# snap-research/F8Net

Hardware: AMD Instinct MI355X
Metric: images/sec at bs=128 (ResNet-50 INT8) (higher is better)
Workload: dtype int8 x int8 -> int32 (exact integer)

## Files before the change

f8net_amd/_lib.py:

```python
import ctypes
import os

_HERE = os.path.dirname(os.path.abspath(__file__))
LIB_PATH = os.environ.get('F8NET_LIB') or os.path.join(_HERE, 'libf8net.so')

F8_OK = 0


class F8Error(RuntimeError):
    def __init__(self, status, msg):
        super().__init__(f'libf8net: {msg} (status {status})')
        self.status = status


class ConvDesc(ctypes.Structure):
    _fields_ = [(n, ctypes.c_int32) for n in
                ('cin', 'cout', 'kernel', 'stride', 'pad', 'groups', 'weight_fl', 'input_fl',
                 'input_signed', 'quant_input', 'relu')]


class LinearDesc(ctypes.Structure):
    _fields_ = [(n, ctypes.c_int32) for n in
                ('in_features', 'out_features', 'weight_fl', 'input_fl', 'input_signed', 'quant_input')]

# ... 25 lines not shown
    ('f8_net_num_launches', _i, [_vp]),
    ('f8_net_arena_bytes', _sz, [_vp]),
    ('f8_net_weight_bytes', _sz, [_vp]),
    ('f8_net_output_fraclen', _i, [_vp]),
    ('f8_net_output_elems', _sz, [_vp]),
    ('f8_net_upload', _i, [_vp]),
    ('f8_net_num_parts', _i, [_vp, _i]),
    ('f8_net_step_launches', _i, [_vp, _i, _i]),
    ('f8_net_run', _i, [_vp, _vp, _vp, _i, _vp]),
    ('f8_net_run_f32', _i, [_vp, _vp, _i, _vp, _i, _vp]),
    ('f8_net_run_u8', _i, [_vp, _vp, _i, _i, ctypes.POINTER(ctypes.c_float), ctypes.POINTER(ctypes.c_float), _vp, _i, _vp]),
    ('f8_net_run_profiled', _i, [_vp, _vp, _vp, _i, _vp, ctypes.POINTER(ctypes.c_float), _i]),
    ('f8_net_launch_info', _i, [_vp, _i, _i, ctypes.c_char_p, _sz, ctypes.POINTER(ctypes.c_double),
                                ctypes.POINTER(ctypes.c_double)]),
    ('f8_net_launch_kernel', _i, [_vp, _i, ctypes.c_char_p, _sz]),
    ('f8_net_launch_valu', _i, [_vp, _i, _i, ctypes.POINTER(ctypes.c_double)]),
    ('f8_net_set_label', _i, [_vp, _i, ctypes.c_char_p]),
    ('f8_net_set_pipelined', _i, [_vp, _i]),
    ('f8_net_autotune', _i, [_vp, _i, _vp]),
    ('f8_net_set_option', _i, [_vp, ctypes.c_char_p, _i]),
    ('f8_net_get_option', _i, [_vp, ctypes.c_char_p, ctypes.POINTER(_i)]),
    ('f8_net_set_input_ready', _i, [_vp, _vp]),
    ('f8_net_check', _i, [_vp]),
]


def lib():
    global _lib
    if _lib is None:
        if not os.path.exists(LIB_PATH):
# ... 18 lines not shown
```

f8net_amd/csrc/f8_chain.hip:

```cpp
#include "f8_device.h"
#include <cstdio>
#include <cstdlib>

namespace f8 {

template <int C, int MID, int W, int H, int R, int CIN0, bool BROT_ = false, bool ALIAS_ = false>
struct ChainCfg {
    static constexpr bool BROT = BROT_, ALIAS = ALIAS_;
    static constexpr int BSLOTS = BROT ? 2 : kChainMaxBlocks;
    static constexpr int T = (H + R - 1) / R;
    static constexpr int PX = R * W, NPT = (PX + 31) / 32, ROWS = NPT * 32;
    static constexpr int PW = W + 2, PR = R + 2;
    static constexpr int XS = C + 16, MS = MID + 16, IS = CIN0 + 16;
    static constexpr int X8_BYTES = ROWS * XS;
    static constexpr int PATCH_BYTES = (PR * PW * MS + 255) / 256 * 256;
    static constexpr int MID2_BYTES = ROWS * MS;
    static constexpr int XIN_BYTES = CIN0 != C ? ROWS * IS : 0;
    static constexpr int BIAS_INTS = 2 * MID + C;
    static constexpr int BIAS_BYTES = (BSLOTS * BIAS_INTS + (CIN0 != C ? C : 0)) * 4;
    static constexpr int MISC_BYTES = 256;
    static_assert(!ALIAS || XIN_BYTES <= PATCH_BYTES, "ALIAS: the shortcut's operand fits the patch");
    static constexpr int LDS_BYTES = X8_BYTES + PATCH_BYTES + MID2_BYTES + (ALIAS ? 0 : XIN_BYTES) + BIAS_BYTES + MISC_BYTES;
    static constexpr int ROWB = W * MID;
    static_assert(LDS_BYTES <= 160 * 1024, "LDS");
    static_assert(X8_BYTES < 65536 + 4096 && PATCH_BYTES < 65536 && MID2_BYTES < 65536, "immediate offsets");
    static_assert(ROWB / 16 <= 256 && (size_t)512 * 4 * ROWB <= kChainXchgBytes, "one 16-byte piece of a halo row per thread of a half workgroup");
};

template <int FAST, bool ACC = false>
__device__ __forceinline__ v4i quant_tile16(const v16i& y, int n, int lo, int hi, unsigned x_or) {
    unsigned d[4];
    const float sc = FAST == 1 ? requant_u8_scale(n) : 0.0f;
#pragma unroll
    for (int g = 0; g < 4; ++g) {
        if constexpr (FAST == 1) d[g] = requant_u8x4(y[4 * g], y[4 * g + 1], y[4 * g + 2], y[4 * g + 3], sc) ^ x_or;
        else if constexpr (FAST == 2) d[g] = requant_u8x4_int(y[4 * g], y[4 * g + 1], y[4 * g + 2], y[4 * g + 3], n) ^ x_or;
        else d[g] = pack4(requant1(y[4 * g], n, lo, hi), requant1(y[4 * g + 1], n, lo, hi), requant1(y[4 * g + 2], n, lo, hi), requant1(y[4 * g + 3], n, lo, hi)) ^ x_or;
    }
    auto s0 = __builtin_amdgcn_permlane32_swap(d[0], d[2], false, false);
// ... 27 lines not shown
#ifndef F8_CH_PRIO
#define F8_CH_PRIO 0
#endif
#ifndef F8_CH_BREG
#define F8_CH_BREG 1
#endif
    constexpr bool EARLY = F8_CH_EARLY != 0 && T > 1 && !ROT;
#ifndef F8_CH_SPLIT
#define F8_CH_SPLIT 1
#endif
#ifndef F8_CH_HALO_AUX
#define F8_CH_HALO_AUX 17
#endif
    constexpr int PG_ = NW / (MID / 32), NPW_ = ((R * W + 31) / 32 + PG_ - 1) / PG_;
    constexpr bool SPLIT = F8_CH_SPLIT != 0 && EARLY && PG_ >= 2 && T * R == H && W <= NPW_ * 32 && (R - 1) * W >= NPW_ * 32;
    static_assert(NB <= CM && CM % NB == 0 && NK1 % NB == 0, "a batch of K steps stays inside one 3x3 tap / one weight tile");
    static_assert(!DS0 || KS % NB == 0, "stage-opening block: whole batches");
    static_assert(!ROT || (NK1 % 8 == 0 && CM == 8), "rotation: groups of 8 K steps (256 bytes of a row), whole taps");
    static_assert(WSTAT || NPT == 2, "streamed P3: exactly one pixel pair");
    static_assert(W <= 62, "tile");

    if constexpr (FAST == 1) set_fp_round_nearest_even();
    extern __shared__ __attribute__((aligned(16))) char lds[];
    char* const x8 = lds;
    char* const patch = x8 + Cfg::X8_BYTES;
    char* const mid2 = patch + Cfg::PATCH_BYTES;
    char* const xin = Cfg::ALIAS ? patch : mid2 + Cfg::MID2_BYTES;
    int* const bias_lds = (int*)(mid2 + Cfg::MID2_BYTES + (Cfg::ALIAS ? 0 : Cfg::XIN_BYTES));
    int* const misc = bias_lds + Cfg::BIAS_BYTES / 4;

// ... 31 lines not shown
    auto bias_store = [&](int b, const int (&v)[NBI]) {
        int tb = tid; asm volatile("" : "+v"(tb));
#pragma unroll
        for (int k = 0; k < NBI; ++k) if (tb + k * NT < BIAS_INTS) bias_lds[(b & 1) * BIAS_INTS + tb + k * NT] = v[k];
    };
    if constexpr (!BROT) {
        for (int b = 0; b < a.nblk; ++b) {
            const ChainBlk& B = a.blk[b];
            for (int i = tid; i < BIAS_INTS; i += NT)
                bias_lds[b * BIAS_INTS + i] = i < 2 * MID ? ((TAIL && b == 0) ? 0 : (i < MID ? B.b0[i] : B.b2[i - MID])) : B.b4[i - 2 * MID];
        }
    }
    if constexpr (DS0) for (int i = tid; i < C; i += NT) bias_lds[BSLOTS * BIAS_INTS + i] = a.blk[0].bsc[i];
    __syncthreads();
    const int L = __builtin_amdgcn_readfirstlane(misc[0]);
    const int grp = L / T, ti = L - grp * T;
    const int p0 = ti * R;
    const int rows = (H - p0) < R ? (H - p0) : R;
    const int npx = rows * W;
    const bool has_up = ti > 0, has_dn = ti < T - 1;
    const int rot = ROT ? __builtin_amdgcn_readfirstlane(L * 5 + wave * 3) : 0;

    unsigned* const flags = a.sync + 16;
    const unsigned long long t_limit = (unsigned long long)a.timeout_ticks;
#ifdef F8_TRACE
    unsigned long long tt[16] = {}; unsigned long long t_prev = __builtin_readcyclecounter();
#define F8_CT(i) do { const unsigned long long now_ = __builtin_readcyclecounter(); tt[i] += now_ - t_prev; t_prev = now_; } while (0)
#else
#define F8_CT(i)
#endif

    const int mt = wave & (CM - 1), pg = wave / CM;
    v16i res[NPT][CTW];
    v4i wbuf[NBUF][NB];
    unsigned seq = 0;
// ... 38 lines not shown
            const int f = BI * NB + s, I = f / (NPAIR * KT2), k = f % KT2;
            dst[s] = k < KS ? ldw(wsc, (I * KS + k) * 1024, (unsigned)(wave * CTW * KS * 1024) + wl) : ldw(w4, (I * KK + (k - KS)) * 1024, (unsigned)(wave * CTW * KK * 1024) + wl);
        }
    };
    auto pin = [](auto& xf) {
#pragma unroll
        for (int j = 0; j < (int)(sizeof(xf) / sizeof(xf[0])); ++j) asm volatile("" : "+v"(xf[j]));
    };

    constexpr int CHX = CIN0 / 16, CHM = MID / 16;
    constexpr int NXI = DS0 ? (NPT * 32 * CHX + NT - 1) / NT : 0, NMI = TAIL ? (NPT * 32 * CHM + NT - 1) / NT : 0;
    v4i vin[NXI + NMI > 0 ? NXI + NMI : 1];
    auto in_issue = [&](int n, bool live) {
        if constexpr (DS0) {
            int tq0 = tid; asm volatile("" : "+v"(tq0));
            const int mt0 = (n * H + p0) * W;
#pragma unroll
            for (int k = 0; k < NXI; ++k) {
                const int idx = tq0 + k * NT, row = idx / CHX, c16 = idx % CHX;
                vin[k] = v4i{0, 0, 0, 0};
                if constexpr (TAIL) {
                    const int pr = row / W, pc = row - pr * W;
                    if (live && row < npx) vin[k] = *(const v4i*)(a.x8in + ((size_t)(n * 2 * H + 2 * (p0 + pr)) * (2 * W) + 2 * pc) * CIN0 + c16 * 16);
                } else {
                    if (live && row < npx) vin[k] = *(const v4i*)(a.x8in + (size_t)(mt0 + row) * CIN0 + c16 * 16);
                }
            }
#pragma unroll
            for (int k = 0; k < NMI; ++k) {
                const int idx = tq0 + k * NT, row = idx / CHM, c16 = idx % CHM;
                vin[NXI + k] = v4i{0, 0, 0, 0};
                if (live && row < npx) vin[NXI + k] = *(const v4i*)(a.m2in + (size_t)(mt0 + row) * MID + c16 * 16);
            }
        }
    };
    auto in_commit = [&]() {
        if constexpr (DS0) {
            int tq0 = tid; asm volatile("" : "+v"(tq0));
#pragma unroll
            for (int k = 0; k < NXI; ++k) { const int idx = tq0 + k * NT; if (idx < NPT * 32 * CHX) *(v4i*)(xin + (idx / CHX) * IS + (idx % CHX) * 16) = vin[k]; }
#pragma unroll
            for (int k = 0; k < NMI; ++k) { const int idx = tq0 + k * NT; if (idx < NPT * 32 * CHM) *(v4i*)(mid2 + (idx / CHM) * MS + (idx % CHM) * 16) = vin[NXI + k]; }
        }
    };
#ifndef F8_CH_PREFETCH
#define F8_CH_PREFETCH 1
#endif
    if (F8_CH_PREFETCH) in_issue(grp < a.N ? grp : 0, grp < a.N);

    for (int n = grp; n < a.N; n += a.NG) {
        const int m_tile = (n * H + p0) * W;
        if (!F8_CH_PREFETCH) in_issue(n, true);

        if constexpr (TAIL) {
            static_assert(KT2 % NB == 0 && KS % NB == 0 && NPT % 2 == 0, "TAIL: whole batches per K loop, pixel-tile pairs");
            int bv0[NBI], bv1[NBI];
            if constexpr (BROT) { bias_fetch(0, bv0); bias_fetch(a.nblk > 1 ? 1 : 0, bv1); }
            { F8_LANES; static_for<(NBUF - 1 < NBT ? NBUF - 1 : NBT)>([&](auto bc) { constexpr int Bi = decltype(bc)::value; wt_load(a.blk[0].wsc, a.blk[0].w4, wbuf[Bi], bc, wl16); }); }
            if constexpr (BROT) { bias_store(0, bv0); bias_store(1, bv1); }
            in_commit();
        } else if constexpr (!DS0) {
            F8_LANES;
            const ChainBlk& B0 = a.blk[0];
            const __amdgpu_buffer_rsrc_t rxr = __builtin_amdgcn_make_buffer_rsrc((void*)a.xr, 0, (unsigned)(((a.N * H * W + 31) & ~31) * C * 4), 0x00020000);
#pragma unroll
            for (int pt = 0; pt < NPT; ++pt) {
// ... 79 lines not shown
#define F8_CH_BFILL 1
#endif
                    {
                        const v4i zv = {(int)xor1, (int)xor1, (int)xor1, (int)xor1};
                        if constexpr (F8_CH_BFILL) {
                            constexpr int RB = PW * MS, CPM = MS / 16;
                            for (int o = tq_ * 16; o < RB; o += NT * 16) *(v4i*)(patch + o) = zv;
                            for (int o = (rows + 1) * RB + tq_ * 16; o < Cfg::PR * RB; o += NT * 16) *(v4i*)(patch + o) = zv;
                            if (tq_ < rows * 2 * CPM) {
                                const int r = tq_ / (2 * CPM), q = tq_ - r * 2 * CPM, sidec = q / CPM, c16 = q - sidec * CPM;
                                *(v4i*)(patch + ((r + 1) * PW + (sidec ? PW - 1 : 0)) * MS + c16 * 16) = zv;
                            }
                        } else {
                            for (int o = tq_ * 16; o < Cfg::PATCH_BYTES; o += NT * 16) *(v4i*)(patch + o) = zv;
                        }
                    }
                    v16i acc[NPW];
#pragma unroll
                    for (int g = 0; g < 4; ++g) {
                        const v4i bv = *(const v4i*)(bl + mt * 32 + 8 * g + 4 * lh);
#pragma unroll
                        for (int j = 0; j < NPW; ++j)
#pragma unroll
                            for (int e = 0; e < 4; ++e) acc[j][4 * g + e] = bv[e];
                    }
                    F8_CT(6);
                    constexpr int NBAT1 = NK1B / NB;
                    const char* const xsrc = DSB ? xin : x8;
                    auto rd = [&](v4i (&xf)[NPW], auto gc) {
                        constexpr int G = decltype(gc)::value;
// ... 130 lines not shown
                            for (int e = 0; e < 4; ++e) acc[j][4 * g + e] = bv[e];
                    }
                    unsigned bpb[NPW];
#pragma unroll
                    for (int j = 0; j < NPW; ++j) {
                        const int pix = p12_pix[j], oc = pix < npx ? pix : npx - 1;
                        const int orow = oc / W, ocol = oc - orow * W;
                        bpb[j] = (unsigned)((orow * PW + ocol) * MS + lh * 16);
                    }
                    v4i xfa[NPW], xfb[NPW];
                    constexpr int GH = SPLIT ? 6 * CM : (EARLY ? 3 * CM : NK2 + 1);
                    const int ord = (SPLIT && !((pg + 1) * NPW * 32 > (R - 1) * W)) ? 1 : 0;
                    unsigned bpb2[NPW], bpb3[NPW];
#pragma unroll
                    for (int j = 0; j < NPW; ++j) { bpb2[j] = bpb[j] + (unsigned)(ord ? 2 * PW * MS : 0); bpb3[j] = bpb[j] + (unsigned)(ord ? 0 : 2 * PW * MS); }
                    auto rd = [&](v4i (&xf)[NPW], auto gc) {
                        constexpr int G = decltype(gc)::value, TAP0 = G / CM, CI = G % CM;
                        if constexpr (SPLIT) {
                            constexpr int GRP = TAP0 / 3, DX = TAP0 % 3;
#pragma unroll
                            for (int j = 0; j < NPW; ++j) {
                                if constexpr (GRP == 0) xf[j] = *(const v4i*)(patch + bpb[j] + (PW + DX) * MS + CI * 32);
                                else if constexpr (GRP == 1) xf[j] = *(const v4i*)(patch + bpb2[j] + DX * MS + CI * 32);
                                else xf[j] = *(const v4i*)(patch + bpb3[j] + DX * MS + CI * 32);
                            }
                        } else {
                            constexpr int TAP = EARLY ? (TAP0 < 3 ? TAP0 + 3 : (TAP0 < 6 ? TAP0 - 3 : TAP0)) : TAP0;
                            if constexpr (ROT) {
                                const int tp = tap_of(TAP);
                                const int tr = tp / 3, ts = tp - tr * 3;
                                const unsigned eo = (unsigned)((tr * PW + ts) * MS + CI * 32);
#pragma unroll
                                for (int j = 0; j < NPW; ++j) xf[j] = *(const v4i*)(patch + bpb[j] + eo);
                            } else {
#pragma unroll
                                for (int j = 0; j < NPW; ++j) xf[j] = *(const v4i*)(patch + bpb[j] + ((TAP / 3) * PW + TAP % 3) * MS + CI * 32);
                            }
                        }
                    };
                    rd(xfa, std::integral_constant<int, 0>{});
                    static_for<NK2>([&](auto gc) {
                        constexpr int G = decltype(gc)::value, Bi = G / NB, S = G % NB;
                        if constexpr (S == 0 && Bi + NBUF - 1 < NBAT2) w2_load(pw2, wbuf[(Bi + NBUF - 1) % NBUF], Bi + NBUF - 1, wl16, ord);
                        v4i (&cur)[NPW] = (G & 1) ? xfb : xfa;
                        v4i (&nxt)[NPW] = (G & 1) ? xfa : xfb;
                        if constexpr (G == GH) { F8_CT(3); consume(); F8_CT(2); rd(cur, gc); }
                        if constexpr (G + 1 < NK2 && G + 1 != GH) rd(nxt, std::integral_constant<int, G + 1>{});
                        pin(cur);
#pragma unroll
                        for (int j = 0; j < NPW; ++j) acc[j] = __builtin_amdgcn_mfma_i32_32x32x32_i8(wbuf[Bi % NBUF][S], cur[j], acc[j], 0, 0, 0);
                    });
// ... 182 lines not shown
            }
        };
#ifndef F8_CH_PEEL_LAST
#define F8_CH_PEEL_LAST 1
#endif
        if constexpr (TAIL) block(0, std::integral_constant<int, 2>{}, std::integral_constant<int, 2>{});
        else if constexpr (DS0) block(0, std::integral_constant<int, 1>{}, std::integral_constant<int, 2>{});
        if constexpr (F8_CH_PEEL_LAST) {
            const int b0 = DS0 ? 1 : 0;
            for (int b = b0; b + 1 < a.nblk; ++b) block(b, std::integral_constant<int, 0>{}, std::integral_constant<int, 0>{});
            if (a.nblk > b0) block(a.nblk - 1, std::integral_constant<int, 0>{}, std::integral_constant<int, 1>{});
        } else {
            for (int b = DS0 ? 1 : 0; b < a.nblk; ++b) block(b, std::integral_constant<int, 0>{}, std::integral_constant<int, 2>{});
        }

        if (F8_CH_PREFETCH) in_issue(n + a.NG < a.N ? n + a.NG : n, n + a.NG < a.N);
        if (a.q[0].ptr) {
            constexpr int CH = C / 16;
            int tq1 = tid; asm volatile("" : "+v"(tq1));
            for (int idx = tq1; idx < npx * CH; idx += NT) {
                const int row = idx / CH, c16 = idx % CH;
                const v4i v = *(const v4i*)(x8 + row * XS + c16 * 16);
                *(v4i*)(a.q[0].ptr + (size_t)(m_tile + row) * C + c16 * 16) = v;
            }
        }
        __syncthreads();
        F8_CT(5);
    }
    if (tid == 0) {
        asm volatile("s_waitcnt vmcnt(0)" ::: "memory");
        misc[2] = (__hip_atomic_fetch_add(a.sync + 1, 1u, __ATOMIC_RELAXED, __HIP_MEMORY_SCOPE_AGENT) == gridDim.x - 1u) ? 1 : 0;
// ... 33 lines not shown
void chain_shape(int C, int MID, int H, int W, int cin0, bool tail, int* R, int* wg_per_cu) {
    *R = 4; *wg_per_cu = 1;
    if (F8_CH_R2_S0 && !tail && C == 256 && MID == 64 && H == 56 && W == 56 && cin0 == 64) { *R = 2; *wg_per_cu = 2; }
    if (chain_nw(C, MID, H, W, cin0, tail) == 4) { *R = 2; *wg_per_cu = 2; }
}

template <int C, int MID, int W, int H, int R, int CIN0, int NB, int NBUF, int FAST, bool ROT, bool TAIL = false, int NW = 8>
static hipError_t launch_chain_t(const ChainArgs& a, hipStream_t s) {
    using Cfg = ChainCfg<C, MID, W, H, R, CIN0, TAIL || R < 4, TAIL && NW == 4>;
    static unsigned long long attr_done = 0; int attr_dev = -1;
    if (!dyn_lds_opted_in(&attr_done, &attr_dev)) {
        hipError_t e = hipFuncSetAttribute((const void*)chain_kernel<C, MID, W, H, R, CIN0, NB, NBUF, FAST, ROT, TAIL, NW>, hipFuncAttributeMaxDynamicSharedMemorySize, Cfg::LDS_BYTES);
        if (e != hipSuccess) return e;
        if (attr_dev >= 0) attr_done |= 1ull << attr_dev;
    }
    const int grid = a.NG * Cfg::T;
    if (grid < 1 || grid > (R < 4 ? 512 : 256)) return hipErrorInvalidValue;
#ifdef F8_TRACE
    static unsigned long long* tbuf = nullptr; static int count = 0;
    static const int want = [] { const char* e = getenv("F8_TRACE_CHAIN"); return e ? atoi(e) : -1; }();
    ChainArgs b = a;
    const bool tracing = (count++ == want);
    if (tracing) { if (!tbuf) (void)hipMalloc((void**)&tbuf, (size_t)1 << 19); (void)hipMemsetAsync(tbuf, 0, (size_t)grid * 1024, s); b.trace = tbuf; }
    hipLaunchKernelGGL((chain_kernel<C, MID, W, H, R, CIN0, NB, NBUF, FAST, ROT, TAIL, NW>), dim3(grid), dim3(NW * 64), Cfg::LDS_BYTES, s, b);
    if (tracing) {
        (void)hipStreamSynchronize(s);
        static unsigned long long hb[256 * 8 * 16];
        (void)hipMemcpy(hb, tbuf, (size_t)grid * 1024, hipMemcpyDeviceToHost);
        double ph[16] = {}, pw[8][16] = {}; int n = 0;
        for (int i = 0; i < grid; ++i) {
            ++n;
// ... 36 lines not shown
        if (!(a.q[0].n > 0 && a.q[0].n <= 30 && a.q[0].lo == 0)) return 0;
        f16 = f16 && a.q[0].n <= kRequantU8MaxShift;
    }
    return (a.rq_int || !a.acc_ok || !a.stream_ok || !f16) ? 2 : 1;
}

#define F8_STR2(...) #__VA_ARGS__
#define F8_STR(...) F8_STR2(__VA_ARGS__)
static bool chain_rot(int H, bool tail) {
#ifdef F8_CH_ROT
    return H == 14 && !tail;
#else
    (void)H; (void)tail; return false;
#endif
}
int chain_kernel_name(char* buf, size_t cap, int C, int MID, int H, int W, int cin0, bool tail, int fast) {
    if (cchain_supported(C, MID, H, W, cin0, tail)) return cchain_kernel_name(buf, cap, fast);
    int R = 4, wg = 1;
    chain_shape(C, MID, H, W, cin0, tail, &R, &wg);
    const char* nb = MID == 64 ? F8_STR(F8_CH_S0) : (MID == 128 ? F8_STR(F8_CH_S1) : F8_STR(F8_CH_S2));
    return snprintf(buf, cap, "f8::chain_kernel<%d, %d, %d, %d, %d, %d, %s, %d, %s, %s, %d>", C, MID, W, H, R, cin0, nb, fast, chain_rot(H, tail) ? "true" : "false", tail ? "true" : "false",
                    chain_nw(C, MID, H, W, cin0, tail));
}

hipError_t launch_chain(const ChainArgs& a, int fast, int C, int MID, int H, int W, int cin0, hipStream_t s) {
    if (a.nblk < 1 || a.nblk > kChainMaxBlocks) return hipErrorInvalidValue;
    if (cchain_supported(C, MID, H, W, cin0, a.tail != 0)) return launch_cchain(a, fast, s);
#define F8_CHAIN_INST(...) (fast == 1 ? launch_chain_t<__VA_ARGS__, 1, F8_CHAIN_ROT>(a, s) : fast == 2 ? launch_chain_t<__VA_ARGS__, 2, F8_CHAIN_ROT>(a, s) : launch_chain_t<__VA_ARGS__, 0, F8_CHAIN_ROT>(a, s))
#define F8_CHAIN_ROT false
#if F8_CH_R2_S0
// ... 37 lines not shown
```

f8net_amd/csrc/f8_internal.h:

```cpp
#pragma once
#include <hip/hip_runtime.h>
#include <stdint.h>
#include <stddef.h>

namespace f8 {

struct Options {
    int split = 2;
    int fuse_blocks = 1;
    int fuse_stages = -1;
    int fuse_dual = 1;
    int fuse_ds = 1;
    int fuse_opener = 1;
    int fuse_fc = 1;
    int fuse_stem = 1;
    int fuse_input = 1;
    int wstat = 1;
    int wstat_min_tiles = 2;
    int wstat_fast = 1;
    int s2wreg = 1;
    int wreg = 1;
    int fuse_bchain = 2;
    int fuse_chain = 1;
    int fuse_chain7 = 1;
    int fuse_pool = 1;
    int fuse_tail = 1;
    int chain_timeout_ms = 10000;
    int fuse_p12 = 1;
    int fuse_head2 = 1;
    int fuse_ir = 1;
    int fuse_irchain = 0;
    int patch3x3 = 1;
    int dual_wide = 2048;
    int deep_nk = 7;
    int bk128 = 0;
    int dw_dot4 = 1;
    int dw_mma = 1;
    int stem_rows = 1;
    int stem_grid_div = 0;
    int stem_wpc = 3;
    int opener_stg = 1;
    int chunk56 = -1, chunk28 = -1, chunk14 = -1;
// ... 137 lines not shown

    const int32_t* xr;
    const int8_t* x8in;
    const int8_t* m2in; int32_t tail;
    int32_t N, NG;
    int32_t* out32; QuantOut q[2];
    uint32_t* sync;
    uint32_t* err;
    uint32_t* err_host;
    uint32_t epoch;
    int8_t* xchg;
    uint32_t timeout_ticks;
    void* trace;
    int32_t R;
    int32_t pool;
};
constexpr int kChainSyncWords = 16 + 512;
constexpr int kChainErrWord = 1000;
constexpr size_t kChainXchgBytes = (size_t)512 * 2 * 2 * 3584;

struct BChainBlk {
    const int8_t* wa; const int8_t* wb;
    const int32_t* ba; const int32_t* bb;
    int32_t nq, loq, hiq; uint32_t xorq;
    int32_t n1, lo1, hi1; uint32_t xor1;
    int32_t relu_a, relu1;
    int32_t acc_shl, res_shl;
};
constexpr int kBChainMaxBlocks = 6;
struct BChainArgs {
// ... 94 lines not shown
int conv_inst(const ConvArgs& a, const ConvTile& t, bool res, bool dual, int deep_nk);
int conv_kernel_name(char* buf, size_t cap, const ConvArgs& a, const ConvTile& t, int inst);
hipError_t launch_conv(const ConvArgs& a, const ConvTile& t, int inst, hipStream_t s);
hipError_t launch_fused_bottleneck(const FusedArgs& a, hipStream_t s);
int fused_bottleneck_kernel_name(char* buf, size_t cap, const FusedArgs& a);
bool fused_bottleneck_supported(int C, int MID, int H, int W, int imgs_per_launch, int stage_mask, int* R);
bool fused_ds_supported(int C, int MID, int COUT, int H, int W, int* R);
bool fused_opener_supported(int C, int MID, int COUT, int H, int W, int* R);
int fused_opener_inst(const FusedArgs& a, bool stg);
int fused_opener_kernel_name(char* buf, size_t cap, const FusedArgs& a, int inst);
hipError_t launch_fused_opener(const FusedArgs& a, int inst, hipStream_t s);
bool chain_supported(int C, int MID, int H, int W, int cin0);
bool chain_tail_supported(int C, int MID, int H, int W, int cin0);
int chain_max_blocks(int C, int MID, int H, int W, int cin0, bool tail);
void chain_shape(int C, int MID, int H, int W, int cin0, bool tail, int* R, int* wg_per_cu);
hipError_t launch_chain(const ChainArgs& a, int fast, int C, int MID, int H, int W, int cin0, hipStream_t s);
int chain_kernel_name(char* buf, size_t cap, int C, int MID, int H, int W, int cin0, bool tail, int fast);
bool cchain_supported(int C, int MID, int H, int W, int cin0, bool tail);
size_t cchain_xchg_bytes();
int cchain_clusters(int N, int slots);
int cchain_kernel_name(char* buf, size_t cap, int fast);
int chain_fast(const ChainArgs& a, unsigned shortcut_blocks, bool q8);
hipError_t launch_cchain(const ChainArgs& a, int fast, hipStream_t s);
bool bchain_supported(int C, int H, int W);
bool bchain_ds_supported(int C, int H, int W);
int bchain_tiles_per_img(int C, int H, int W);
hipError_t launch_bchain(const BChainArgs& a, int fast, int C, int H, int W, hipStream_t s);
int bchain_fast(const BChainArgs& a, bool ds, bool q8);
int bchain_kernel_name(char* buf, size_t cap, int C, int H, int W, bool ds, int fast);
bool fused_p12_supported(int C, int MID, int H, int W);
// ... 61 lines not shown
```

f8net_amd/csrc/f8_net.cpp:

```cpp
#include "../../include/f8net.h"
#include "f8_internal.h"

#include <algorithm>
#include <cstdarg>
#include <cstdio>
#include <cstdlib>
#include <cstring>
#include <new>
#include <variant>
#include <string>
#include <mutex>
#include <vector>

using namespace f8;

namespace {

thread_local std::string g_err;

int fail(int code, const char* fmt, ...) {
    char buf[512];
    va_list ap;
    va_start(ap, fmt);
    vsnprintf(buf, sizeof buf, fmt, ap);
// ... 236 lines not shown
    {"fuse_ds", "F8_FUSE_DS", &Options::fuse_ds, 0, 1, true},
    {"fuse_opener", "F8_FUSE_OPENER", &Options::fuse_opener, 0, 1, true},
    {"fuse_fc", "F8_FUSE_FC", &Options::fuse_fc, 0, 1, true},
    {"fuse_stem", "F8_FUSE_STEM", &Options::fuse_stem, 0, 1, true},
    {"fuse_input", "F8_FUSE_INPUT", &Options::fuse_input, 0, 1, true},
    {"fuse_ir", "F8_FUSE_IR", &Options::fuse_ir, 0, 2, true},
    {"fuse_irchain", "F8_FUSE_IRCHAIN", &Options::fuse_irchain, 0, 1, true},
    {"fuse_head2", "F8_FUSE_HEAD2", &Options::fuse_head2, 0, 1, true},
    {"fuse_p12", "F8_FUSE_P12", &Options::fuse_p12, 0, 1, true},
    {"fuse_chain", "F8_FUSE_CHAIN", &Options::fuse_chain, 0, 1, true},
    {"fuse_tail", "F8_FUSE_TAIL", &Options::fuse_tail, 0, 1, true},
    {"fuse_chain7", "F8_FUSE_CHAIN7", &Options::fuse_chain7, 0, 1, true},
    {"fuse_pool", "F8_FUSE_POOL", &Options::fuse_pool, 0, 1, true},
    {"fuse_bchain", "F8_FUSE_BCHAIN", &Options::fuse_bchain, 0, 2, true},
    {"chain_timeout_ms", "F8_CHAIN_TIMEOUT_MS", &Options::chain_timeout_ms, 0, 1 << 20, false},
    {"wreg", "F8_WREG", &Options::wreg, 0, 1, true},
    {"s2wreg", "F8_S2WREG", &Options::s2wreg, 0, 1, true},
    {"wstat", "F8_WSTAT", &Options::wstat, 0, 1, true},
    {"wstat_min_tiles", "F8_WSTAT_MIN_TILES", &Options::wstat_min_tiles, 0, 1 << 20, true},
    {"wstat_fast", "F8_WSTAT_FAST", &Options::wstat_fast, 0, 1, true},
    {"patch3x3", "F8_PATCH3X3", &Options::patch3x3, 0, 1, true},
    {"dual_wide", "F8_DUAL_WIDE", &Options::dual_wide, 0, 1 << 30, true},
    {"deep_nk", "F8_DEEP_NK", &Options::deep_nk, 1, 1 << 20, true},
    {"bk128", "F8_BK128", &Options::bk128, 0, 1, true},
    {"dw_dot4", "F8_DW_DOT4", &Options::dw_dot4, 0, 1, true},
    {"dw_mma", "F8_DW_MMA", &Options::dw_mma, 0, 1, true},
    {"stem_wpc", "F8_STEM_WPC", &Options::stem_wpc, 1, 8, false},
    {"stem_rows", "F8_STEM_ROWS", &Options::stem_rows, 0, 1, true},
    {"stem_grid_div", "F8_STEM_GRID_DIV", &Options::stem_grid_div, 0, 32, false},
    {"opener_stg", "F8_OPENER_STG", &Options::opener_stg, 0, 1, true},
// ... 1880 lines not shown
                B.relu_a = na.cd.relu; B.relu_b = nb.cd.relu; B.relu1 = ND[hh.fused_add].relu;
                if (k == 0) { a.acc_ok = 1; a.rq_int = rq_int; a.stream_ok = (hds || stream_bounded(net, na.a)) ? 1 : 0; }
                a.acc_ok = a.acc_ok && conv_acc_bounded(na) && conv_acc_bounded(nb);
                a.stream_ok = a.stream_ok && stream_bounded(net, ND[hh.fused_add].out);
                const int dfl = T[hh.out].fl - (hds ? T[ng.out].fl : T[na.a].fl);
                B.acc_shl = dfl < 0 ? -dfl : 0; B.res_shl = dfl > 0 ? dfl : 0;
            }
            const Node& hf = ND[ch[0]];
            const bool tail = hf.tail, ds = hf.fbd_a >= 0 || tail;
            const Node& a0 = tail ? ND[hf.dual] : ND[ds ? hf.fbd_a : hf.fb_a];
            const Tensor& oT = T[ND[nd.fused_add].out];
            a.tail = tail ? 1 : 0;
            a.pool = nd.pool >= 0 ? 1 : 0;
            st.C = oT.C; st.MID = tail ? a0.cd.cin : a0.cd.cout; st.H = oT.H; st.W = oT.W; st.cin0 = tail ? hf.cd.cin : a0.cd.cin;
            chain_shape(st.C, st.MID, st.H, st.W, st.cin0, tail, &a.R, &st.wg_per_cu);
            st.tiles = (st.H + a.R - 1) / a.R;
            st.cluster = (!ds || tail) && cchain_supported(st.C, st.MID, st.H, st.W, st.cin0, tail);
            out_formats(a.q);
            st.inst = chain_fast(a, shortcut_blocks, nq > 0);
            chain_kernel_name(kb, sizeof kb, st.C, st.MID, st.H, st.W, st.cin0, tail, st.inst);
            st.args = a; break;
        }
        case S_BCHAIN: {
            const std::vector<int>& ch = nd.bchain;
            BChainArgs a{};
            a.nblk = (int)ch.size();
            const bool ds = ND[ch[0]].bds_a >= 0;
            for (int k = 0; k < a.nblk; ++k) {
                const Node& hk = ND[ch[k]];
                const bool hds = hk.bds_a >= 0;
                const Node& c2 = hds ? ND[hk.bds_b] : hk; Node& c1 = ND[hds ? hk.bds_a : hk.bb_a];
                BChainBlk& B = a.blk[k];
// ... 233 lines not shown
            if ((e = hipMalloc((void**)&net->d_chain, net->chain_stride * parts_cap)) != hipSuccess) return hip_fail(e, "hipMalloc(chain scratch)");
            if ((e = hipMemset(net->d_chain, 0, net->chain_stride * parts_cap)) != hipSuccess) return hip_fail(e, "hipMemset(chain scratch)");
            if (hipHostMalloc((void**)&net->h_err, 64, hipHostMallocMapped) == hipSuccess) {
                *net->h_err = 0u;
                if (hipHostGetDevicePointer((void**)&net->h_err_dev, net->h_err, 0) != hipSuccess) { (void)hipHostFree(net->h_err); net->h_err = nullptr; net->h_err_dev = nullptr; }
            } else { net->h_err = nullptr; (void)hipGetLastError(); }
        }
    for (int p = 0; p < parts_cap; ++p)
        if (net->stem_zero_bytes && (e = hipMemset(net->d_arena + p * net->arena_stride + net->stem_zero_off, net->stem_zero_val, net->stem_zero_bytes)) != hipSuccess)
            return hip_fail(e, "hipMemset(stem halo)");
    if ((e = hipDeviceSynchronize()) != hipSuccess) return hip_fail(e, "upload sync");
    net->uploaded = true;
    return F8_OK;
}

static int chain_launch_groups(const f8_net* net, const Step& st, int N) {
    const int slots = (net->num_cu > 0 ? std::min(net->num_cu, 256) : 256) * st.wg_per_cu;
    if (slots < st.tiles) {
        fail(F8_ERR_STATE, "f8_net_run: a stage-chain launch needs %d co-resident workgroups per image, the device has %d compute units (plan with fuse_chain = 0 / fuse_bchain = 0)", st.tiles, net->num_cu);
        return 0;
    }
    if (!st.cluster) return chain_groups(N, slots / st.tiles);
    const int ng = cchain_clusters(N, slots);
    if (ng < 1) fail(F8_ERR_STATE, "f8_net_run: the 7x7 stage-chain launch needs 8 co-resident workgroups, the device has %d compute units (plan with fuse_chain7 = 0)", net->num_cu);
    return ng;
}

static int run_step(const f8_net* net, const Step& st, const int32_t* input, void* output, int n0, int N, int c0, int part, hipStream_t s) {
    const auto& T = net->tensors;
    char* A = net->d_arena + (size_t)part * net->arena_stride;
    auto fp = [&](const Form& F) -> char* { return A + F.off + (size_t)c0 * F.bytes_per_img; };
    const Node& nd = net->nodes[st.node];
    auto fill_out = [&](int32_t** out32, QuantOut q[2]) {
        if (st.out.t < 0 || st.dense) return;
        const Tensor& o = T[st.out.t];
        if (st.out.f32 >= 0) *out32 = (int32_t*)fp(o.forms[st.out.f32]);
        for (int k = 0; k < 2; ++k) if (st.out.f8[k] >= 0) q[k].ptr = (int8_t*)fp(o.forms[st.out.f8[k]]);
    };
    char* const chain = net->d_chain ? net->d_chain + (size_t)part * net->chain_stride : nullptr;
    const uint32_t* chain_err = chain ? (const uint32_t*)chain + kChainErrWord : nullptr;
// ... 66 lines not shown
            const Form& xF = T[st.src_t].forms[st.src_f];
            FusedArgs a = std::get<FusedArgs>(st.args);
            a.x8 = (const int8_t*)fp(xF); a.x_bytes = (uint32_t)(xF.bytes_per_img * N); a.N = N;
            if (st.kind == S_FUSED && nd.fbd_a < 0) a.xr = (const int32_t*)fp(T[st.res_t].forms[st.res_f]);
            fill_out(&a.out32, a.q);
            if (st.kind == S_P12) e = nd.p12_s2 ? launch_fused_opener(a, st.inst, s) : launch_fused_p12(a, s);
            else e = (nd.fbd_a >= 0 && nd.fbd_s2) ? launch_fused_opener(a, st.inst, s) : launch_fused_bottleneck(a, s);
            break;
        }
        case S_CHAIN: {
            ChainArgs a = std::get<ChainArgs>(st.args);
            const Form& xF = T[st.src_t].forms[st.src_f];
            if (a.tail || net->nodes[nd.chain[0]].fbd_a >= 0) a.x8in = (const int8_t*)fp(xF); else a.xr = (const int32_t*)fp(xF);
            if (a.tail) a.m2in = (const int8_t*)fp(T[st.src2_t].forms[st.src2_f]);
            a.N = N;
            if ((a.NG = chain_launch_groups(net, st, N)) < 1) return F8_ERR_STATE;
            fill_out(&a.out32, a.q);
            if (const int rc = chain_scratch(a)) return rc;
            e = launch_chain(a, st.inst, st.C, st.MID, st.H, st.W, st.cin0, s);
            break;
        }
        case S_BCHAIN: {
            BChainArgs a = std::get<BChainArgs>(st.args);
            const Tensor& xs = T[st.src_t];
            if (net->nodes[nd.bchain[0]].bds_a >= 0) { a.x8in = (const int8_t*)fp(xs.forms[st.src_f]); a.x8sc = (const int8_t*)fp(xs.forms[st.res_f]); }
            else a.xr = (const int32_t*)fp(xs.forms[st.src_f]);
            a.N = N;
            if ((a.NG = chain_launch_groups(net, st, N)) < 1) return F8_ERR_STATE;
            fill_out(&a.out32, a.q);
            if (const int rc = chain_scratch(a)) return rc;
            e = launch_bchain(a, st.inst, st.C, st.H, st.W, s);
            break;
        }
        case S_IR: {
            const Tensor& x = T[st.src_t];
            IRArgs a = std::get<IRArgs>(st.args);
            a.x8 = (const int8_t*)fp(x.forms[st.src_f]); a.N = N;
            if (st.res_t >= 0) a.xr = (const int32_t*)fp(T[st.res_t].forms[st.res_f]);
            fill_out(&a.out32, a.q);
            e = launch_fused_ir(a, x.Cs, nd.coutP, st.inst, s);
            break;
        }
        case S_IRCHAIN: {
// ... 471 lines not shown
```

f8net_amd/net.py:

```python
import ctypes

import numpy as np

from . import _lib, topology
from ._lib import ConvDesc, LinearDesc, check

AVGPOOL_SHIFT = 6


def _np_i32(a):
    return np.ascontiguousarray(np.asarray(a), dtype=np.int32)


class F8Net:

    def __init__(self):
        self._L = _lib.lib()
        self._h = self._L.f8_net_create()
        if not self._h:
            raise MemoryError('f8_net_create failed')
        self.max_batch = 0
        self.out_elems = 0
        self.out_float = True
        self.in_shape = None
# ... 93 lines not shown
    def num_parts(self, N):
        return check(self._L.f8_net_num_parts(self._h, int(N)))

    def step_launches(self, i, N):
        return check(self._L.f8_net_step_launches(self._h, i, int(N)))

    def launch_valu(self, i, N):
        v = ctypes.c_double(0.0)
        check(self._L.f8_net_launch_valu(self._h, i, int(N), ctypes.byref(v)))
        return v.value

    def launch_kernel(self, i):
        buf = ctypes.create_string_buffer(256)
        check(self._L.f8_net_launch_kernel(self._h, i, buf, 256))
        return buf.value.decode()

    def upload(self):
        check(self._L.f8_net_upload(self._h))

    def _check_input(self, x):
        import torch
        if not x.is_cuda:
            raise ValueError('F8Net.run: input must be a CUDA/HIP tensor (there is no CPU path)')
        if x.dtype != torch.int32 or not x.is_contiguous():
            raise ValueError('F8Net.run: input must be contiguous int32 NCHW')
        if tuple(x.shape[1:]) != tuple(self.in_shape):
            raise ValueError(f'F8Net.run: input shape {tuple(x.shape)} != [N,{self.in_shape}]')
        if not (1 <= x.shape[0] <= self.max_batch):
            raise ValueError(f'F8Net.run: batch {x.shape[0]} outside [1,{self.max_batch}]')

# ... 154 lines not shown
```

include/f8net.h:

```cpp
#ifndef F8NET_H
#define F8NET_H

#include <stddef.h>
#include <stdint.h>

#ifdef __cplusplus
extern "C" {
#endif

#define F8NET_VERSION 200

typedef enum f8_status {
    F8_OK = 0,
    F8_ERR_INVALID = -1,
    F8_ERR_UNSUPPORTED = -2,
    F8_ERR_HIP = -3,
    F8_ERR_NOMEM = -4,
    F8_ERR_STATE = -5
} f8_status;

const char* f8_status_string(int status);
const char* f8_last_error(void);
int f8_version(void);
int f8_device_count(void);
// ... 80 lines not shown
int f8_net_set_option(f8_net* net, const char* key, int value);
int f8_net_get_option(const f8_net* net, const char* key, int* value);

int f8_net_num_parts(const f8_net* net, int N);

int f8_net_step_launches(const f8_net* net, int i, int N);

int f8_net_run_profiled(f8_net* net, const int32_t* input_dev, void* output_dev, int N,
                        void* stream, float* ms, int cap);

int f8_net_launch_info(const f8_net* net, int i, int N, char* name, size_t name_cap,
                       double* alg_bytes, double* alg_ops);

int f8_net_launch_valu(const f8_net* net, int i, int N, double* essential_lane_ops);
int f8_net_launch_kernel(const f8_net* net, int i, char* buf, size_t cap);

int f8_net_set_label(f8_net* net, int t, const char* label);

#ifdef __cplusplus
}
#endif
#endif
```

Baseline: 152,500.

## Stack image pairs in chain kernel to eliminate ragged row tiles

When H is not a multiple of the tile row count R but 2H is, the stage-chain kernel now treats two images as one stacked 2H-row tensor, so tiles fill completely instead of leaving a partial last tile per image. A zero-pad LDS region and per-pixel tap base redirection keep the 3x3 convolution from reading across the image seam, and odd batches use a ragged final tile. This is meant to cut wasted MFMA work and workgroups on partial tiles, at the cost of extra address logic and LDS. The behaviour is on by default via a new chain_stack option, and a launch-grid query API is added.

```diff
diff --git a/f8net_amd/_lib.py b/f8net_amd/_lib.py
--- a/f8net_amd/_lib.py
+++ b/f8net_amd/_lib.py
@@ -63,6 +63,7 @@
     ('f8_net_launch_info', _i, [_vp, _i, _i, ctypes.c_char_p, _sz, ctypes.POINTER(ctypes.c_double),
                                 ctypes.POINTER(ctypes.c_double)]),
     ('f8_net_launch_kernel', _i, [_vp, _i, ctypes.c_char_p, _sz]),
+    ('f8_net_launch_grid', _i, [_vp, _i, _i, _i] + [ctypes.POINTER(_i)] * 4),
     ('f8_net_launch_valu', _i, [_vp, _i, _i, ctypes.POINTER(ctypes.c_double)]),
     ('f8_net_set_label', _i, [_vp, _i, ctypes.c_char_p]),
     ('f8_net_set_pipelined', _i, [_vp, _i]),
diff --git a/f8net_amd/csrc/f8_chain.hip b/f8net_amd/csrc/f8_chain.hip
--- a/f8net_amd/csrc/f8_chain.hip
+++ b/f8net_amd/csrc/f8_chain.hip
@@ -8,7 +8,13 @@
 struct ChainCfg {
     static constexpr bool BROT = BROT_, ALIAS = ALIAS_;
     static constexpr int BSLOTS = BROT ? 2 : kChainMaxBlocks;
+#ifdef F8_CH_ABL_NORAG
+    static constexpr int T = H / R;
+#else
     static constexpr int T = (H + R - 1) / R;
+#endif
+    static constexpr bool STACKABLE = H % R != 0 && (2 * H) % R == 0;
+    static constexpr int T2 = STACKABLE ? 2 * H / R : T;
     static constexpr int PX = R * W, NPT = (PX + 31) / 32, ROWS = NPT * 32;
     static constexpr int PW = W + 2, PR = R + 2;
     static constexpr int XS = C + 16, MS = MID + 16, IS = CIN0 + 16;
@@ -20,9 +26,11 @@
     static constexpr int BIAS_BYTES = (BSLOTS * BIAS_INTS + (CIN0 != C ? C : 0)) * 4;
     static constexpr int MISC_BYTES = 256;
     static_assert(!ALIAS || XIN_BYTES <= PATCH_BYTES, "ALIAS: the shortcut's operand fits the patch");
-    static constexpr int LDS_BYTES = X8_BYTES + PATCH_BYTES + MID2_BYTES + (ALIAS ? 0 : XIN_BYTES) + BIAS_BYTES + MISC_BYTES;
+    static constexpr int ZPAD_BYTES = STACKABLE ? 3 * MS : 0;
+    static constexpr int ZPAD_OFF = X8_BYTES + PATCH_BYTES + MID2_BYTES + (ALIAS ? 0 : XIN_BYTES) + BIAS_BYTES + MISC_BYTES;
+    static constexpr int LDS_BYTES = ZPAD_OFF + ZPAD_BYTES;
     static constexpr int ROWB = W * MID;
-    static_assert(LDS_BYTES <= 160 * 1024, "LDS");
+    static_assert(LDS_BYTES <= 160 * 1024 && ZPAD_OFF % 16 == 0, "LDS");
     static_assert(X8_BYTES < 65536 + 4096 && PATCH_BYTES < 65536 && MID2_BYTES < 65536, "immediate offsets");
     static_assert(ROWB / 16 <= 256 && (size_t)512 * 4 * ROWB <= kChainXchgBytes, "one 16-byte piece of a halo row per thread of a half workgroup");
 };
@@ -80,6 +88,7 @@
 #endif
     constexpr int PG_ = NW / (MID / 32), NPW_ = ((R * W + 31) / 32 + PG_ - 1) / PG_;
     constexpr bool SPLIT = F8_CH_SPLIT != 0 && EARLY && PG_ >= 2 && T * R == H && W <= NPW_ * 32 && (R - 1) * W >= NPW_ * 32;
+    static_assert(!(Cfg::STACKABLE && SPLIT), "the seam's tap bases live in the plain EARLY tap order");
     static_assert(NB <= CM && CM % NB == 0 && NK1 % NB == 0, "a batch of K steps stays inside one 3x3 tap / one weight tile");
     static_assert(!DS0 || KS % NB == 0, "stage-opening block: whole batches");
     static_assert(!ROT || (NK1 % 8 == 0 && CM == 8), "rotation: groups of 8 K steps (256 bytes of a row), whole taps");
@@ -141,11 +150,16 @@
     if constexpr (DS0) for (int i = tid; i < C; i += NT) bias_lds[BSLOTS * BIAS_INTS + i] = a.blk[0].bsc[i];
     __syncthreads();
     const int L = __builtin_amdgcn_readfirstlane(misc[0]);
-    const int grp = L / T, ti = L - grp * T;
+    constexpr bool STACKABLE = Cfg::STACKABLE && !ROT;
+    const bool stk2 = STACKABLE && a.stack == 2;
+    const int TC = stk2 ? Cfg::T2 : T, HS = stk2 ? 2 * H : H;
+    const int grp = L / TC, ti = L - grp * TC;
     const int p0 = ti * R;
-    const int rows = (H - p0) < R ? (H - p0) : R;
-    const int npx = rows * W;
-    const bool has_up = ti > 0, has_dn = ti < T - 1;
+    const int n_end = !stk2 ? a.N : ((a.N & 1) && p0 >= H ? a.N / 2 : (a.N + 1) / 2);
+    auto ragged = [&](int n) { return STACKABLE && HS != H && 2 * n + 1 == a.N && p0 == (H / R) * R; };
+    const int rows0 = (HS - p0) < R ? (HS - p0) : R;
+    const int npx0 = rows0 * W;
+    const bool has_up = ti > 0, has_dn0 = ti < TC - 1;
     const int rot = ROT ? __builtin_amdgcn_readfirstlane(L * 5 + wave * 3) : 0;
 
     unsigned* const flags = a.sync + 16;
@@ -214,14 +228,20 @@
     auto in_issue = [&](int n, bool live) {
         if constexpr (DS0) {
             int tq0 = tid; asm volatile("" : "+v"(tq0));
-            const int mt0 = (n * H + p0) * W;
+            const int mt0 = (n * HS + p0) * W;
+            const int npx = ragged(n) ? (H - p0) * W : npx0;
 #pragma unroll
             for (int k = 0; k < NXI; ++k) {
                 const int idx = tq0 + k * NT, row = idx / CHX, c16 = idx % CHX;
                 vin[k] = v4i{0, 0, 0, 0};
                 if constexpr (TAIL) {
                     const int pr = row / W, pc = row - pr * W;
-                    if (live && row < npx) vin[k] = *(const v4i*)(a.x8in + ((size_t)(n * 2 * H + 2 * (p0 + pr)) * (2 * W) + 2 * pc) * CIN0 + c16 * 16);
+                    if constexpr (STACKABLE) {
+                        const int g = mt0 / W + pr, img = g / H, y = g - img * H;
+                        if (live && row < npx) vin[k] = *(const v4i*)(a.x8in + ((size_t)(img * 2 * H + 2 * y) * (2 * W) + 2 * pc) * CIN0 + c16 * 16);
+                    } else {
+                        if (live && row < npx) vin[k] = *(const v4i*)(a.x8in + ((size_t)(n * 2 * H + 2 * (p0 + pr)) * (2 * W) + 2 * pc) * CIN0 + c16 * 16);
+                    }
                 } else {
                     if (live && row < npx) vin[k] = *(const v4i*)(a.x8in + (size_t)(mt0 + row) * CIN0 + c16 * 16);
                 }
@@ -246,10 +266,13 @@
 #ifndef F8_CH_PREFETCH
 #define F8_CH_PREFETCH 1
 #endif
-    if (F8_CH_PREFETCH) in_issue(grp < a.N ? grp : 0, grp < a.N);
-
-    for (int n = grp; n < a.N; n += a.NG) {
-        const int m_tile = (n * H + p0) * W;
+    if (F8_CH_PREFETCH) in_issue(grp < n_end ? grp : 0, grp < n_end);
+
+    for (int n = grp; n < n_end; n += a.NG) {
+        const int m_tile = (n * HS + p0) * W;
+        const bool rag = ragged(n);
+        const int rows = rag ? H - p0 : rows0, npx = rag ? (H - p0) * W : npx0;
+        const bool has_dn = has_dn0 && !rag;
         if (!F8_CH_PREFETCH) in_issue(n, true);
 
         if constexpr (TAIL) {
@@ -359,6 +382,7 @@
                         } else {
                             for (int o = tq_ * 16; o < Cfg::PATCH_BYTES; o += NT * 16) *(v4i*)(patch + o) = zv;
                         }
+                        if constexpr (STACKABLE) { if (tq_ < Cfg::ZPAD_BYTES / 16) *(v4i*)(lds + Cfg::ZPAD_OFF + tq_ * 16) = zv; }
                     }
                     v16i acc[NPW];
 #pragma unroll
@@ -519,6 +543,17 @@
                     unsigned bpb2[NPW], bpb3[NPW];
 #pragma unroll
                     for (int j = 0; j < NPW; ++j) { bpb2[j] = bpb[j] + (unsigned)(ord ? 2 * PW * MS : 0); bpb3[j] = bpb[j] + (unsigned)(ord ? 0 : 2 * PW * MS); }
+                    unsigned bpbt[NPW], bpbb[NPW];
+#pragma unroll
+                    for (int j = 0; j < NPW; ++j) {
+                        bpbt[j] = bpb[j]; bpbb[j] = bpb[j];
+                        if constexpr (STACKABLE) {
+                            const int pix = p12_pix[j], srow = p0 + (pix < npx ? pix : npx - 1) / W;
+                            const unsigned zo = (unsigned)(Cfg::ZPAD_OFF - Cfg::X8_BYTES + lh * 16);
+                            if (srow == H) bpbt[j] = zo;
+                            if (srow == H - 1) bpbb[j] = zo - (unsigned)(2 * PW * MS);
+                        }
+                    }
                     auto rd = [&](v4i (&xf)[NPW], auto gc) {
                         constexpr int G = decltype(gc)::value, TAP0 = G / CM, CI = G % CM;
                         if constexpr (SPLIT) {
@@ -539,7 +574,7 @@
                                 for (int j = 0; j < NPW; ++j) xf[j] = *(const v4i*)(patch + bpb[j] + eo);
                             } else {
 #pragma unroll
-                                for (int j = 0; j < NPW; ++j) xf[j] = *(const v4i*)(patch + bpb[j] + ((TAP / 3) * PW + TAP % 3) * MS + CI * 32);
+                                for (int j = 0; j < NPW; ++j) xf[j] = *(const v4i*)(patch + (TAP < 3 ? bpbt[j] : TAP < 6 ? bpb[j] : bpbb[j]) + ((TAP / 3) * PW + TAP % 3) * MS + CI * 32);
                             }
                         }
                     };
@@ -752,7 +787,7 @@
             for (int b = DS0 ? 1 : 0; b < a.nblk; ++b) block(b, std::integral_constant<int, 0>{}, std::integral_constant<int, 2>{});
         }
 
-        if (F8_CH_PREFETCH) in_issue(n + a.NG < a.N ? n + a.NG : n, n + a.NG < a.N);
+        if (F8_CH_PREFETCH) in_issue(n + a.NG < n_end ? n + a.NG : n, n + a.NG < n_end);
         if (a.q[0].ptr) {
             constexpr int CH = C / 16;
             int tq1 = tid; asm volatile("" : "+v"(tq1));
@@ -816,7 +851,9 @@
         if (e != hipSuccess) return e;
         if (attr_dev >= 0) attr_done |= 1ull << attr_dev;
     }
-    const int grid = a.NG * Cfg::T;
+    const bool stk2 = a.stack == 2;
+    if (stk2 && (!Cfg::STACKABLE || ROT)) return hipErrorInvalidValue;
+    const int grid = a.NG * (stk2 ? Cfg::T2 : Cfg::T);
     if (grid < 1 || grid > (R < 4 ? 512 : 256)) return hipErrorInvalidValue;
 #ifdef F8_TRACE
     static unsigned long long* tbuf = nullptr; static int count = 0;
@@ -883,6 +920,12 @@
     (void)H; (void)tail; return false;
 #endif
 }
+bool chain_stackable(int C, int MID, int H, int W, int cin0, bool tail) {
+    if (cchain_supported(C, MID, H, W, cin0, tail) || chain_rot(H, tail)) return false;
+    int R = 4, wg = 1;
+    chain_shape(C, MID, H, W, cin0, tail, &R, &wg);
+    return H % R != 0 && (2 * H) % R == 0;
+}
 int chain_kernel_name(char* buf, size_t cap, int C, int MID, int H, int W, int cin0, bool tail, int fast) {
     if (cchain_supported(C, MID, H, W, cin0, tail)) return cchain_kernel_name(buf, cap, fast);
     int R = 4, wg = 1;
diff --git a/f8net_amd/csrc/f8_internal.h b/f8net_amd/csrc/f8_internal.h
--- a/f8net_amd/csrc/f8_internal.h
+++ b/f8net_amd/csrc/f8_internal.h
@@ -26,6 +26,7 @@
     int fuse_pool = 1;
     int fuse_tail = 1;
     int chain_timeout_ms = 10000;
+    int chain_stack = 1;
     int fuse_p12 = 1;
     int fuse_head2 = 1;
     int fuse_ir = 1;
@@ -193,6 +194,7 @@
     void* trace;
     int32_t R;
     int32_t pool;
+    int32_t stack;
 };
 constexpr int kChainSyncWords = 16 + 512;
 constexpr int kChainErrWord = 1000;
@@ -317,6 +319,7 @@
 bool chain_tail_supported(int C, int MID, int H, int W, int cin0);
 int chain_max_blocks(int C, int MID, int H, int W, int cin0, bool tail);
 void chain_shape(int C, int MID, int H, int W, int cin0, bool tail, int* R, int* wg_per_cu);
+bool chain_stackable(int C, int MID, int H, int W, int cin0, bool tail);
 hipError_t launch_chain(const ChainArgs& a, int fast, int C, int MID, int H, int W, int cin0, hipStream_t s);
 int chain_kernel_name(char* buf, size_t cap, int C, int MID, int H, int W, int cin0, bool tail, int fast);
 bool cchain_supported(int C, int MID, int H, int W, int cin0, bool tail);
diff --git a/f8net_amd/csrc/f8_net.cpp b/f8net_amd/csrc/f8_net.cpp
--- a/f8net_amd/csrc/f8_net.cpp
+++ b/f8net_amd/csrc/f8_net.cpp
@@ -274,6 +274,7 @@
     {"fuse_pool", "F8_FUSE_POOL", &Options::fuse_pool, 0, 1, true},
     {"fuse_bchain", "F8_FUSE_BCHAIN", &Options::fuse_bchain, 0, 2, true},
     {"chain_timeout_ms", "F8_CHAIN_TIMEOUT_MS", &Options::chain_timeout_ms, 0, 1 << 20, false},
+    {"chain_stack", "F8_CHAIN_STACK", &Options::chain_stack, 0, 1, true},
     {"wreg", "F8_WREG", &Options::wreg, 0, 1, true},
     {"s2wreg", "F8_S2WREG", &Options::s2wreg, 0, 1, true},
     {"wstat", "F8_WSTAT", &Options::wstat, 0, 1, true},
@@ -2184,8 +2185,9 @@
             a.pool = nd.pool >= 0 ? 1 : 0;
             st.C = oT.C; st.MID = tail ? a0.cd.cin : a0.cd.cout; st.H = oT.H; st.W = oT.W; st.cin0 = tail ? hf.cd.cin : a0.cd.cin;
             chain_shape(st.C, st.MID, st.H, st.W, st.cin0, tail, &a.R, &st.wg_per_cu);
-            st.tiles = (st.H + a.R - 1) / a.R;
             st.cluster = (!ds || tail) && cchain_supported(st.C, st.MID, st.H, st.W, st.cin0, tail);
+            a.stack = (net->opt.chain_stack && !st.cluster && chain_stackable(st.C, st.MID, st.H, st.W, st.cin0, tail)) ? 2 : 1;
+            st.tiles = (a.stack * st.H + a.R - 1) / a.R;
             out_formats(a.q);
             st.inst = chain_fast(a, shortcut_blocks, nq > 0);
             chain_kernel_name(kb, sizeof kb, st.C, st.MID, st.H, st.W, st.cin0, tail, st.inst);
@@ -2449,16 +2451,38 @@
     return F8_OK;
 }
 
-static int chain_launch_groups(const f8_net* net, const Step& st, int N) {
-    const int slots = (net->num_cu > 0 ? std::min(net->num_cu, 256) : 256) * st.wg_per_cu;
-    if (slots < st.tiles) {
-        fail(F8_ERR_STATE, "f8_net_run: a stage-chain launch needs %d co-resident workgroups per image, the device has %d compute units (plan with fuse_chain = 0 / fuse_bchain = 0)", st.tiles, net->num_cu);
-        return 0;
-    }
-    if (!st.cluster) return chain_groups(N, slots / st.tiles);
-    const int ng = cchain_clusters(N, slots);
-    if (ng < 1) fail(F8_ERR_STATE, "f8_net_run: the 7x7 stage-chain launch needs 8 co-resident workgroups, the device has %d compute units (plan with fuse_chain7 = 0)", net->num_cu);
-    return ng;
+static int chain_geometry(const Step& st, int N, int num_cu, int32_t* stack, int* tiles) {
+    const int slots = (num_cu > 0 ? std::min(num_cu, 256) : 256) * st.wg_per_cu;
+    *tiles = st.tiles;
+    if (*stack == 2 && slots < st.tiles) {
+        const int R = std::get<ChainArgs>(st.args).R;
+        *stack = 1; *tiles = (st.H + R - 1) / R;
+    }
+    if (slots < *tiles) return 0;
+    if (st.cluster) return cchain_clusters(N, slots);
+    return chain_groups(*stack == 2 ? (N + 1) / 2 : N, slots / *tiles);
+}
+
+static int chain_launch_groups(const f8_net* net, const Step& st, int N, int32_t* stack) {
+    int tiles = 0;
+    const int ng = chain_geometry(st, N, net->num_cu, stack, &tiles);
+    if (ng >= 1) return ng;
+    if (st.cluster) fail(F8_ERR_STATE, "f8_net_run: the 7x7 stage-chain launch needs 8 co-resident workgroups, the device has %d compute units (plan with fuse_chain7 = 0)", net->num_cu);
+    else fail(F8_ERR_STATE, "f8_net_run: a stage-chain launch needs %d co-resident workgroups per image, the device has %d compute units (plan with fuse_chain = 0 / fuse_bchain = 0)", tiles, net->num_cu);
+    return 0;
+}
+
+int f8_net_launch_grid(const f8_net* net, int i, int N, int num_cu, int* tiles, int* groups, int* grid, int* stack) {
+    if (!net || !net->finalized) return fail(F8_ERR_STATE, "f8_net_launch_grid: not finalized");
+    if (i < 0 || i >= (int)net->steps.size() || N < 1 || !tiles || !groups || !grid || !stack) return fail(F8_ERR_INVALID, "f8_net_launch_grid: index / batch / null pointer");
+    const Step& st = net->steps[i];
+    *tiles = *groups = *grid = *stack = 0;
+    if (st.kind != S_CHAIN && st.kind != S_BCHAIN) return F8_OK;
+    int32_t sk = st.kind == S_CHAIN ? std::get<ChainArgs>(st.args).stack : 1;
+    *groups = chain_geometry(st, N, num_cu, &sk, tiles);
+    *stack = sk < 1 ? 1 : sk;
+    *grid = *groups * (st.cluster ? 8 : *tiles);
+    return F8_OK;
 }
 
 static int run_step(const f8_net* net, const Step& st, const int32_t* input, void* output, int n0, int N, int c0, int part, hipStream_t s) {
@@ -2555,7 +2579,7 @@
             if (a.tail || net->nodes[nd.chain[0]].fbd_a >= 0) a.x8in = (const int8_t*)fp(xF); else a.xr = (const int32_t*)fp(xF);
             if (a.tail) a.m2in = (const int8_t*)fp(T[st.src2_t].forms[st.src2_f]);
             a.N = N;
-            if ((a.NG = chain_launch_groups(net, st, N)) < 1) return F8_ERR_STATE;
+            if ((a.NG = chain_launch_groups(net, st, N, &a.stack)) < 1) return F8_ERR_STATE;
             fill_out(&a.out32, a.q);
             if (const int rc = chain_scratch(a)) return rc;
             e = launch_chain(a, st.inst, st.C, st.MID, st.H, st.W, st.cin0, s);
@@ -2567,7 +2591,7 @@
             if (net->nodes[nd.bchain[0]].bds_a >= 0) { a.x8in = (const int8_t*)fp(xs.forms[st.src_f]); a.x8sc = (const int8_t*)fp(xs.forms[st.res_f]); }
             else a.xr = (const int32_t*)fp(xs.forms[st.src_f]);
             a.N = N;
-            if ((a.NG = chain_launch_groups(net, st, N)) < 1) return F8_ERR_STATE;
+            { int32_t one = 1; if ((a.NG = chain_launch_groups(net, st, N, &one)) < 1) return F8_ERR_STATE; }
             fill_out(&a.out32, a.q);
             if (const int rc = chain_scratch(a)) return rc;
             e = launch_bchain(a, st.inst, st.C, st.H, st.W, s);
diff --git a/f8net_amd/net.py b/f8net_amd/net.py
--- a/f8net_amd/net.py
+++ b/f8net_amd/net.py
@@ -131,6 +131,11 @@
         buf = ctypes.create_string_buffer(256)
         check(self._L.f8_net_launch_kernel(self._h, i, buf, 256))
         return buf.value.decode()
+
+    def launch_grid(self, i, N, num_cu=0):
+        v = [ctypes.c_int(0) for _ in range(4)]
+        check(self._L.f8_net_launch_grid(self._h, i, int(N), int(num_cu), *[ctypes.byref(x) for x in v]))
+        return tuple(x.value for x in v)
 
     def upload(self):
         check(self._L.f8_net_upload(self._h))
diff --git a/include/f8net.h b/include/f8net.h
--- a/include/f8net.h
+++ b/include/f8net.h
@@ -118,6 +118,7 @@
 
 int f8_net_launch_valu(const f8_net* net, int i, int N, double* essential_lane_ops);
 int f8_net_launch_kernel(const f8_net* net, int i, char* buf, size_t cap);
+int f8_net_launch_grid(const f8_net* net, int i, int N, int num_cu, int* tiles, int* groups, int* grid, int* stack);
 
 int f8_net_set_label(f8_net* net, int t, const char* label);
 
```

Result: faster. 156,800, median of 6 (+2.8%).
